# shaunplee/ray-tracing

Measured on AMD Instinct MI355X. Metric: Msamples/s (WxHxspp/s) + achieved HBM GB/s, final scene 1200x800x500spp, higher is better.
Workload: dtype f64

## Files before the change

include/rt_wide.h:

```cpp
#pragma once
#include <stdint.h>

#define RT_WIDE 4

typedef struct rt_wnode {
  float lo[3][RT_WIDE];
  float hi[3][RT_WIDE];
  int32_t child[RT_WIDE];
  int32_t pad[RT_WIDE];
} rt_wnode;

typedef struct rt_qnode {
  float origin[3];
  float scale[3];
  uint32_t qlo[3];
  uint32_t qhi[3];
  int32_t child[RT_WIDE];
} rt_qnode;

#define RT_WKEY_BITS 14
#define RT_WKEY_MASK ((1u << RT_WKEY_BITS) - 1u)
#define RT_WKEY_MAX_IDS (1 << (RT_WKEY_BITS - 1))
#define RT_WKEY_REJECTED 0x7f800000u

#if defined(__HIPCC__) || defined(__CUDACC__)
#define RT_WKEY_FN __host__ __device__ static inline
#else
#define RT_WKEY_FN static inline
#endif

RT_WKEY_FN int rt_wkey_fits(long long n_wide_nodes, long long n_leaf_slots) {
  return n_wide_nodes <= RT_WKEY_MAX_IDS && n_leaf_slots <= RT_WKEY_MAX_IDS;
}
RT_WKEY_FN int32_t rt_wkey_pack(uint32_t key_bits, int32_t ref) {
  return (int32_t)((key_bits & ~RT_WKEY_MASK) | ((uint32_t)ref & RT_WKEY_MASK));
}
RT_WKEY_FN int32_t rt_wkey_ref(int32_t word) {
  const uint32_t low = (uint32_t)word & RT_WKEY_MASK;
  return (int32_t)(low ^ (1u << (RT_WKEY_BITS - 1))) - (1 << (RT_WKEY_BITS - 1));
}

#ifdef __cplusplus
static_assert(sizeof(rt_wnode) == 128, "rt_wnode is 128 bytes");
static_assert(sizeof(rt_qnode) == 64, "rt_qnode is 64 bytes");
#endif
```

ray-tracing_amd/csrc/rt_kernels.h:

```cpp
#pragma once
#include <hip/hip_runtime.h>

#include <algorithm>
#include <cstdlib>
#include <cmath>
#include <cstdio>
#include <cstring>
#include <string>
#include <vector>

#include "rt.h"
#include "rt_device.h"
#include "rt_error.h"
#include "rt_internal.h"
#include "rt_trace.h"

using namespace rtd;

namespace {

struct UDiv {
  uint32_t m;
  int s1, s2;
};
// ... 481 lines not shown
          wq[1] = end2;
        }
      }
      if (w < 0) break;
      const uint32_t pid = (uint32_t)((long long)row * L.W + px);
      g.init(A.seed, pid, (uint32_t)s);
      g.reserve(3);
      const double ru = g.draw(), rv = g.draw();
      const int y = L.H - 1 - row;
      const double u = ((double)px + ru) / (double)L.W;
      const double v = ((double)y + rv) / (double)L.H;
      const Ray cray = get_ray(L.cam, u, v, g);
      t.ray.o = cray.o;
      t.ray.d = cray.d;
      t.ray.tm = cray.tm;
      thr = v3(1.0, 1.0, 1.0);
      depth = L.max_depth;
      if (depth <= 0) {
        end_sample(vmul(v3(1.0, 1.0, 1.0), v3(0.0, 0.0, 0.0)));
        continue;
      }
      start = true;
      if constexpr ((F & F_COUNT) != 0) ++segs;
    }
    if (start) {
      trav_begin<F>(t, plain(t.ray), S.world, kEps, INFINITY);
      if (S.ref_walk) trav_restart_ref(t, S.world, INFINITY);
      trav_media_first<F>(S, t, kEps, cnt, g, side);
      walking = true;
    }
    if (!walking) break;
    unsigned long long s1 = 0;
    if constexpr ((F & F_COUNT) != 0) s1 = stamp();
    const int live = __popcll(__ballot(true));
    const int stop = (live * A.trav_stop) >> 6;
    const int ls = (F & F_WIDE) ? A.leaf_stop : A.box_first;
    walk_until<F, PK>(S, t, walking, kEps, stk, stride, joint, stop, (live * ls) >> 6, cnt, g, side, A.med_batch);
    ready = !walking;
    if constexpr ((F & F_COUNT) != 0) {
      const unsigned long long s2 = stamp();
      ph_shade += s0b - s0;
      ph_setup += s1 - s0b;
      ph_trav += s2 - s1;
    }
  }
  if constexpr ((F & F_COUNT) != 0) {
    wave_add(&L.work[0], segs);
    wave_add(&L.work[1], cnt.box);
    wave_add(&L.work[2], cnt.prim);
    wave_add(&L.work[3], cnt.other);
    wave_add(&L.work[4], cnt.light);
    wave_add(&L.work[5], blocks);
    wave_add(&L.work[6], samples);
    wave_add(&L.work[7], cnt.wide);
    wave_add(&L.work[11], cnt.islot);
    wave_add(&L.work[12], cnt.lslot);
    wave_add(&L.work[13], cnt.oslot);
    wave_add(&L.work[14], cnt.phit);
    wave_add(&L.work[15], cnt.ties);
    if ((threadIdx.x & 63) == 0) {
      atomicAdd(&L.work[8], ph_setup);
      atomicAdd(&L.work[9], ph_trav);
      atomicAdd(&L.work[10], ph_shade);
    }
  }
}

template <unsigned F>
constexpr int lane_ints() {
  return ((F & (F_WIDE | F_MIXW)) ? RT_WSTACK : RT_STACK) + ((F & F_FRAMES) ? kSideInts : 0);
}

template <unsigned F, int WAVES>
__global__ void __launch_bounds__(RT_BLOCK, WAVES) render_philox2(RenderArgs A, int stack_entries) {
  extern __shared__ __attribute__((aligned(16))) int stk_mem[];
  __shared__ uint32_t wave_q[RT_BLOCK / 64][2];
  const LaunchConst& L = stage_const(A, stk_mem);
  __syncthreads();
  int* lane0 = &stk_mem[kLcBytes / 4 + threadIdx.x];
  philox_loop2<F>(A, L, A.S, lane0, RT_BLOCK, lane0 + stack_entries * RT_BLOCK,
                  wave_q[__builtin_amdgcn_readfirstlane(threadIdx.x >> 6)]);
}

template <unsigned F, int WAVES, bool LEAF_LDS = false, bool PK = false>
__global__ void __launch_bounds__(WAVES * 256, WAVES)
    render_philox2_lds(RenderArgs A, int n_nodes, int stack_entries, int n_leaves) {
  extern __shared__ __attribute__((aligned(16))) unsigned char lds0[];
  __shared__ uint32_t wave_q[WAVES * 4][2];
  constexpr int rec = (F & F_WIDE) ? (int)sizeof(rt_wnode) : (int)sizeof(rt_node);
  constexpr int lrec = (int)sizeof(rt_node);
  const LaunchConst& L = stage_const(A, lds0);
  unsigned char* lds = lds0 + kLcBytes;
  {
    const uint4* src = (F & F_WIDE) ? reinterpret_cast<const uint4*>(A.S.wnodes)
                                    : reinterpret_cast<const uint4*>(A.S.nodes);
    uint4* dst = reinterpret_cast<uint4*>(lds);
    const int n16 = n_nodes * (rec / 16);
    for (int i = threadIdx.x; i < n16; i += blockDim.x) dst[i] = src[i];
    const uint4* lsrc = reinterpret_cast<const uint4*>(A.S.leaves);
    uint4* ldst = reinterpret_cast<uint4*>(lds + (size_t)n_nodes * rec);
    const int l16 = n_leaves * (lrec / 16);
    for (int i = threadIdx.x; i < l16; i += blockDim.x) ldst[i] = lsrc[i];
  }
  __syncthreads();
  Scene S = A.S;
  if constexpr ((F & F_WIDE) != 0) S.wnodes = reinterpret_cast<const rt_wnode*>(lds);
  else S.nodes = reinterpret_cast<const rt_node*>(lds);
  if constexpr (LEAF_LDS) S.leaves = reinterpret_cast<const rt_node*>(lds + (size_t)n_nodes * rec);
  else n_leaves = 0;
  constexpr int lanes = WAVES * 256;
  unsigned char* lane_base = lds + (size_t)n_nodes * rec + (size_t)n_leaves * lrec;
  int* stk = reinterpret_cast<int*>(lane_base) + threadIdx.x;
  int* side_p = reinterpret_cast<int*>(lane_base + (size_t)stack_entries * lanes * sizeof(int)) + threadIdx.x;
  philox_loop2<F, PK>(A, L, S, stk, lanes, side_p, wave_q[__builtin_amdgcn_readfirstlane(threadIdx.x >> 6)]);
}

template <bool SKIP>
__device__ __forceinline__ void tail_body(const LaunchConst& A) {
  const long long j = (long long)blockIdx.x * 256 + threadIdx.x;
  if (j >= A.items_total - A.tail_start) return;
  int px, row, s0, s1;
  long long slot;
  if (!work_item<SKIP>(A, (uint32_t)(A.tail_start + j), px, row, s0, s1, slot)) return;
  const double* q = A.tail_buf + j * A.chunk * 3;
  V3 sum = v3(0, 0, 0);
  for (int k = 0; k < s1 - s0; ++k) sum = sum + v3(q[3 * k], q[3 * k + 1], q[3 * k + 2]);
  store_partial(A, slot, sum);
}
__global__ void __launch_bounds__(256) tail_combine(LaunchConst A) { tail_body<false>(A); }
__global__ void __launch_bounds__(256) tail_combine_skip(LaunchConst A) { tail_body<true>(A); }

template <bool MOMENTS, bool SKIP = false>
__device__ __forceinline__ void combine_body(const LaunchConst& A, double* moments) {
  const long long idx = (long long)blockIdx.x * 256 + threadIdx.x;
  if (idx >= A.slab) return;
  int px, row;
  if (!work_pixel(A, (uint32_t)idx, px, row)) return;
  if constexpr (SKIP) {
    if (skip_bit(A.skip, (uint32_t)idx)) return;
  }
  V3 acc = (A.combine & 1) ? vload(A.acc + idx * 3) : v3(0, 0, 0);
  V3 mom = v3(0, 0, 0);
  if constexpr (MOMENTS) {
    if (A.combine & 1) mom = vload(moments + idx * 3);
  }
  for (int k = 0; k < A.chunks; ++k) {
    const double* q = A.partial + ((long long)k * A.slab + idx) * 3;
    acc = acc + v3(q[0], q[1], q[2]);
    if constexpr (MOMENTS) {
      const int s0 = (A.chunk_base + k) * A.chunk;
      const double n = (double)(A.spp - s0 < A.chunk ? A.spp - s0 : A.chunk);
      mom = mom + v3((q[0] * q[0]) / n, (q[1] * q[1]) / n, (q[2] * q[2]) / n);
    }
  }
  if constexpr (MOMENTS) {
    moments[idx * 3 + 0] = mom.x;
    moments[idx * 3 + 1] = mom.y;
    moments[idx * 3 + 2] = mom.z;
  }
  if (A.combine & 2) {
    store_pixel(A, idx, divide(acc, (double)A.spp));
  } else {
    A.acc[idx * 3 + 0] = acc.x;
    A.acc[idx * 3 + 1] = acc.y;
    A.acc[idx * 3 + 2] = acc.z;
  }
// ... 579 lines not shown
  }
  if (w == 2) return (const void*)render_philox2_lds<V, 2, false, true>;
  if (w == 4) return (const void*)render_philox2_lds<V, 4, false, true>;
  if (w == 1) return (const void*)render_philox2_lds<V, 1, false, true>;
  return (const void*)render_philox2_lds<V, 3, false, true>;
}
template <unsigned V>
const void* pick_w(bool lds, int w, bool leaf_lds = false, bool q = false, bool pk = false) {
  if constexpr ((V & ~F_SKIP) == (kVarSpheres | F_WIDE)) {
    if (!lds && q) {
      if (w == 2) return (const void*)render_philox2<V | F_QNODE, 2>;
      if (w == 3) return (const void*)render_philox2<V | F_QNODE, 3>;
      if (w == 4) return (const void*)render_philox2<V | F_QNODE, 4>;
      return (const void*)render_philox2<V | F_QNODE, 1>;
    }
  }
  if constexpr ((V & F_WIDE) != 0 && (V & ~F_SKIP) != (kVarSpheres | F_WIDE)) {
    if (lds && pk) return pick_packed<V>(w, leaf_lds);
  }
  if constexpr ((V & F_WIDE) != 0) {
    if (lds && leaf_lds) {
      if (w == 4) return (const void*)render_philox2_lds<V, 4, true>;
      if (w == 2) return (const void*)render_philox2_lds<V, 2, true>;
      if (w == 3) return (const void*)render_philox2_lds<V, 3, true>;
    }
  }
  if (lds) {
    if (w == 2) return (const void*)render_philox2_lds<V, 2>;
    if (w == 4) return (const void*)render_philox2_lds<V, 4>;
    if (w == 1) return (const void*)render_philox2_lds<V, 1>;
    return (const void*)render_philox2_lds<V, 3>;
  }
  if (w == 2) return (const void*)render_philox2<V, 2>;
  if (w == 3) return (const void*)render_philox2<V, 3>;
  if (w == 4) return (const void*)render_philox2<V, 4>;
  return (const void*)render_philox2<V, 1>;
}
template <unsigned V>
const void* pick(int loop, bool lds, int w, bool count, bool leaf_lds, bool q = false, bool skip = false,
                 bool pk = false) {
  if constexpr ((V & F_SKIP) == 0) {
    if (skip) return count ? nullptr : pick<V | F_SKIP>(loop, lds, w, false, leaf_lds, q, false, pk);
    if (count) {
      if constexpr (V == kVarSpheres) {
        if (loop == 2 && q) return (const void*)render_philox2<V | F_WIDE | F_COUNT | F_QNODE, 1>;
      }
      if (loop == 2) return (const void*)render_philox2<V | F_WIDE | F_COUNT, 1>;
      return loop ? (const void*)render_philox2<V | F_COUNT, 1> : (const void*)render_philox<V | F_COUNT, 1>;
    }
  }
  if (loop == 2) return pick_w<V | F_WIDE>(lds, w, leaf_lds, q, pk);
  if (loop == 1) return pick_w<V>(lds, w);
  if (lds) {
    if (w == 2) return (const void*)render_philox_lds<V, 2>;
    if (w == 4) return (const void*)render_philox_lds<V, 4>;
    if (w == 1) return (const void*)render_philox_lds<V, 1>;
    return (const void*)render_philox_lds<V, 3>;
  }
  if (w == 2) return (const void*)render_philox<V, 2>;
  if (w == 3) return (const void*)render_philox<V, 3>;
  if (w == 4) return (const void*)render_philox<V, 4>;
  return (const void*)render_philox<V, 1>;
}
template <unsigned V>
const void* pick_full(int loop, bool lds, int w, bool count, bool skip = false) {
  if constexpr ((V & F_SKIP) == 0) {
    if (skip) return count ? nullptr : pick_full<V | F_SKIP>(loop, lds, w, false);
    if (count) return loop ? (const void*)render_philox2<V | F_COUNT, 1> : (const void*)render_philox<V | F_COUNT, 1>;
  }
  if (loop) {
    if (lds) return w >= 3 ? (const void*)render_philox2_lds<V, 3> : (const void*)render_philox2_lds<V, 2>;
    if (w >= 4) return (const void*)render_philox2<V, 4>;
    return w >= 3 ? (const void*)render_philox2<V, 3> : (const void*)render_philox2<V, 2>;
  }
  return w >= 2 ? (const void*)render_philox<V, 2> : (const void*)render_philox<V, 1>;
}

}

namespace rt {
const void* philox_kernel_spheres(int loop, bool lds, int w, bool count, bool leaf_lds, bool q, bool skip, bool pk);
const void* philox_kernel_spheres_global(int w, bool skip);
const void* philox_kernel_spheres_packed(int w, bool leaf_lds, bool skip);
const void* philox_kernel_cornell(int loop, bool lds, int w, bool count, bool leaf_lds, bool skip, bool pk);
const void* philox_kernel_full(int loop, bool lds, int w, bool count, bool skip);
const void* philox_kernel_full_dark(int loop, bool lds, int w, bool count, bool skip);
}
```

ray-tracing_amd/csrc/rt_render.hip:

```cpp
#include <rccl/rccl.h>

#include <numeric>
#include <vector>

#include "rt_frame_blob.h"
#include "rt_kernels.h"
#include "rt_prepare.h"


struct rt_ctx {
  int device = 0;
  int cu_count = 0;
  int blocks_per_cu = 0;
  hipStream_t stream = nullptr;
  hipEvent_t ev0 = nullptr, ev1 = nullptr;
  hipEvent_t ev_done = nullptr;
  hipStream_t last_stream = nullptr;
  rt_node* d_nodes = nullptr;
  DMat* d_mats = nullptr;
  rt_texture* d_texs = nullptr;
  rt_perlin* d_perlins = nullptr;
  rt_image* d_images = nullptr;
  uint8_t* d_pool = nullptr;
  Scene scene{};
// ... 383 lines not shown
    R.S = A.S;
    R.lc = d_lc;
    R.seed = A.seed;
    R.flags = A.flags;
    R.trav_stop = A.trav_stop;
    R.leaf_stop = A.leaf_stop;
    R.box_first = A.box_first;
    R.med_batch = A.med_batch;
    R.prof = A.prof;
    if (units_of(slab * per_batch) >= (1ll << 32) - (1ll << 24))
      return invalid("image too large: more than 2^32 - 2^24 work units per shard and launch");
    const size_t need_tail = (size_t)std::min(slab * per_batch, tail_items) * (size_t)A.chunk * 3 * sizeof(double);
    if (need_tail > c->tail_bytes) {
      HIPCHK(hipEventSynchronize(c->ev_done));
      (void)hipFree(c->d_tail);
      c->d_tail = nullptr;
      c->tail_bytes = 0;
      ++c->allocs;
      HIPCHK(hipMalloc((void**)&c->d_tail, need_tail));
      c->tail_bytes = need_tail;
    }
    A.tail_buf = c->d_tail;
    for (int b0 = 0; b0 < chunks_total; b0 += per_batch) {
      const int nk = std::min(per_batch, chunks_total - b0);
      const int k0 = span_first + b0;
      fill_batch_geometry(A, k0, nk, tail_items);
      const bool last = b0 + nk == chunks_total;
      A.combine = (k0 > 0 ? 1 : 0) | (last && !span.keep ? 2 : 0);
      {
        LaunchConst B = A;
        void* sargs[] = {&B, &d_lc};
        HIPCHK(hipLaunchKernel((const void*)launch_setup, dim3(1), dim3(64), sargs, 0, st));
        HIPCHK(hipGetLastError());
      }
      if (b0 == 0) HIPCHK(hipEventRecord(ev_begin, st));
      HIPCHK(hipLaunchKernel(fn, grid, block, args, bytes, st));
      HIPCHK(hipGetLastError());
      if (A.tail_start < A.items_total) {
        LaunchConst B = A;
        void* targs[] = {&B};
        HIPCHK(hipLaunchKernel(A.skip ? (const void*)tail_combine_skip : (const void*)tail_combine, dim3((unsigned)((A.items_total - A.tail_start + 255) / 256)),
                               dim3(256), targs, 0, st));
        HIPCHK(hipGetLastError());
      }
      if (last) HIPCHK(hipEventRecord(ev_end, st));
      const int rc = launch_combine(c, A, st, span.moments);
      if (rc) return rc;
    }
    return RT_OK;
  };
  const char* stop_env = std::getenv("RTAMD_TRAV_STOP");
  {
    const char* be = std::getenv("RTAMD_BATCH");
    A.batch = be ? std::max(1, std::min(4096, std::atoi(be))) : 1024;
    const double waves = (double)c->cu_count * 4 * 4;
    A.batch_per_item = (float)(1.0 / (16.0 * waves));
    const char* bf = std::getenv("RTAMD_BATCH_FLOOR");
    A.batch_floor = bf ? std::max(0, std::min(1024, std::atoi(bf))) : (is_full(variant_for(c->features)) ? 0 : 64);
  }
  A.trav_stop = stop_env ? std::max(0, std::min(63, std::atoi(stop_env)))
                         : (c->n_nodes > 20000 ? 16 : 8);
  const char* leaf_env = std::getenv("RTAMD_LEAF_STOP");
  A.leaf_stop = leaf_env ? std::max(0, std::min(64, std::atoi(leaf_env))) : A.trav_stop;
  const char* box_env = std::getenv("RTAMD_BOX_FIRST");
  A.box_first = box_env ? std::max(0, std::min(64, std::atoi(box_env))) : 4;
  const char* med_env = std::getenv("RTAMD_MED_BATCH");
  A.med_batch = med_env ? std::max(0, std::min(64, std::atoi(med_env))) : 0;
  A.rev_tiles = env_off("RTAMD_TILE_REV") || !std::getenv("RTAMD_TILE_REV") ? 0u : (uint32_t)per_shard;
  const unsigned var = variant_for(c->features);
  const bool count = d_work != nullptr;
  const bool skip = A.skip != nullptr;
  if (skip && count) return invalid("the counting build has no adaptive-frame kernels");
  const bool replace = c->replace_ok && !env_off("RTAMD_REPLACE");
  const char* wenv = std::getenv("RTAMD_WIDE");
  const bool want_wide = wenv ? wenv[0] != '0' : c->rebuilt_bvh;
  const bool wide = replace && c->d_wnodes && !(A.flags & RT_FLAG_REFERENCE_CULL) && want_wide && !is_full(var);
  const int loop = wide ? 2 : (replace ? 1 : 0);
  if (loop && is_full(var)) {
    const char* te = std::getenv("RTAMD_TAIL");
    tail_items = (long long)c->cu_count * (te ? std::max(0, std::min(1 << 16, std::atoi(te))) : 768);
  }
  int waves = (var == kVarSpheres || loop) ? waves_target(3) : waves_target(is_full(var) ? 2 : 1);
  const int side_ints = side_ints_of(var, c->scene.frames, loop) + (lane_lds_of(var, loop) ? 4 : 0);
  if (!count && !env_off("RTAMD_LDS") && (!is_full(var) || loop)) {
    const int entries = wide ? c->wide_stack_need + 3 : c->stack_need + 2;
    const int items = wide ? c->n_wnodes : c->n_nodes;
    const size_t rec = wide ? sizeof(rt_wnode) : sizeof(rt_node);
    const bool leaf_lds = wide && !env_off("RTAMD_LEAF_LDS");
    auto lds_bytes = [&](int w, int& n_leaves) {
      const size_t b =
          (size_t)kLcBytes + (size_t)items * rec + (size_t)(entries + side_ints) * (w * 256) * sizeof(int);
      n_leaves = leaf_lds && b + (size_t)c->n_leaves * sizeof(rt_node) <= kLdsBudget ? c->n_leaves : 0;
      return b + (size_t)n_leaves * sizeof(rt_node);
    };
    int n_leaves = 0;
    if (var == kVarSpheres && !std::getenv("RTAMD_WAVES") && lds_bytes(4, n_leaves) <= kLdsBudget &&
        (!leaf_lds || n_leaves > 0) && A.work_total >= (long long)c->cu_count * 1024)
      waves = 4;
    const int block = waves * 256;
    const size_t bytes = lds_bytes(waves, n_leaves);
    if (bytes <= kLdsBudget) {
      const bool pk = wide && wide_keys_packed(c);
      const void* fn = philox_kernel(var, loop, true, waves, false, skip, n_leaves > 0, false, pk);
      c->last_wide_packed = pk;
      HIPCHK(hipFuncSetAttribute(fn, hipFuncAttributeMaxDynamicSharedMemorySize, (int)bytes));
      int n_items = items;
      void* args[] = {&R, &n_items, (void*)&entries, &n_leaves};
      c->last_launch = rt_launch_info{var | (loop == 2 ? F_WIDE : 0u) | (skip ? F_SKIP : 0u), loop, 1, n_leaves > 0, waves, c->cu_count,
                                      block, (int)bytes, A.work_total, A.chunk,
                                      (loop == 2 || (loop == 1 && c->mixed_wide)) ? c->n_wnodes : 0, batches, 0};
      return run(fn, dim3(c->cu_count), dim3(block), bytes, args);
    }
  }
  const void* fn = philox_kernel(var, loop, false, count ? 1 : waves, count, skip, false, loop == 2 && c->d_qnodes);
  c->last_wide_packed = 0;
  int entries = wide ? c->wide_stack_need + 3 : c->stack_need + 2;
  const size_t dyn = loop ? (size_t)kLcBytes + (size_t)(entries + side_ints) * RT_BLOCK * sizeof(int) : 0;
  if (loop) HIPCHK(hipFuncSetAttribute(fn, hipFuncAttributeMaxDynamicSharedMemorySize, (int)dyn));
  int bpc = 1;
  HIPCHK(hipOccupancyMaxActiveBlocksPerMultiprocessor(&bpc, fn, RT_BLOCK, dyn));
  const long long want = (A.work_total + RT_BLOCK - 1) / RT_BLOCK;
  const long long resident = (long long)c->cu_count * std::max(1, bpc);
  const int grid = (int)std::max(1ll, std::min(want, resident));
  c->last_launch = rt_launch_info{var | (loop == 2 ? F_WIDE : 0u) | (count ? F_COUNT : 0u) | (skip ? F_SKIP : 0u), loop, 0, 0,
                                  count ? 1 : waves, grid, RT_BLOCK, (int)dyn, A.work_total, A.chunk,
                                  (loop == 2 || (loop == 1 && c->mixed_wide)) ? c->n_wnodes : 0, batches, 0};
  void* args[] = {&R, &entries};
  return run(fn, dim3(grid), dim3(RT_BLOCK), dyn, args);
}

int render_multi(rt_ctx* c, const rt_camera* cam, rt_render_params p, uint8_t* out_rgb, double* out_lin) {
  const int n = 1 + (int)c->peers.size();
  p.shard_count = n;
  int tile, tiles_x;
  long long tt, ps, slab;
  geometry(&p, tile, tiles_x, tt, ps, slab);
  auto dev_ctx = [&](int r) { return r == 0 ? c : c->peers[r - 1]; };
  const long long npx = (long long)p.width * p.height;
  int rc = RT_OK;
  for (int r = 0; r < n && !rc; ++r) {
    rt_ctx* d = dev_ctx(r);
    DEVICE_SCOPE(d->device);
    if ((rc = grow(d, d->fb_slab, (size_t)slab * 3))) break;
    if (out_lin && (rc = grow(d, d->fb_slab_lin, sizeof(double) * (size_t)slab * 3))) break;
  }
  {
    DEVICE_SCOPE(c->device);
    if (!rc) rc = grow(c, c->fb_gather, (size_t)n * slab * 3);
    if (!rc && out_lin) rc = grow(c, c->fb_gather_lin, sizeof(double) * (size_t)n * slab * 3);
    if (!rc) rc = grow(c, c->fb_img, (size_t)npx * 3);
    if (!rc && out_lin) rc = grow(c, c->fb_img_lin, sizeof(double) * (size_t)npx * 3);
  }
  if (rc) return rc;
  void* gathered = c->fb_gather.p;
  void* gathered_lin = c->fb_gather_lin.p;
  void* img = c->fb_img.p;
  void* img_lin = c->fb_img_lin.p;
  for (int r = 0; r < n; ++r) {
    rt_ctx* d = dev_ctx(r);
    DEVICE_SCOPE(d->device);
    rt_render_params pr = p;
    pr.shard_rank = r;
    if ((rc = launch_philox(d, cam, &pr, r, n, (uint8_t*)d->fb_slab.p, out_lin ? (double*)d->fb_slab_lin.p : nullptr,
                            d->stream)))
      return rc;
    if (r == 0) HIPCHK(hipEventRecord(c->ev_gather, c->stream));
  }
  {
    DeviceGuard _dg(c->device);
    NCCLCHK(ncclGroupStart());
    for (int r = 0; r < n; ++r) {
      rt_ctx* d = dev_ctx(r);
      const ncclResult_t g = ncclGather(d->fb_slab.p, r == 0 ? gathered : nullptr, (size_t)slab * 3, ncclUint8, 0,
                                        c->comms[r], d->stream);
      const ncclResult_t gl = g == ncclSuccess && out_lin
                                  ? ncclGather(d->fb_slab_lin.p, r == 0 ? gathered_lin : nullptr, (size_t)slab * 3,
                                               ncclFloat64, 0, c->comms[r], d->stream)
                                  : g;
      if (gl != ncclSuccess) {
        (void)ncclGroupEnd();
        return nccl_fail(gl, "ncclGather");
      }
    }
    NCCLCHK(ncclGroupEnd());
  }
  {
    DEVICE_SCOPE(c->device);
    HIPCHK(hipEventRecord(c->ev_gathered, c->stream));
    if ((rc = rt_assemble_async(c, &p, (const uint8_t*)gathered, (uint8_t*)img, c->stream))) return rc;
    if (out_lin && (rc = rt_assemble_linear_async(c, &p, (const double*)gathered_lin, (double*)img_lin, c->stream)))
      return rc;
    HIPCHK(hipEventRecord(c->ev_asm, c->stream));
  }
  for (int r = 0; r < n; ++r) {
    rt_ctx* d = dev_ctx(r);
    DEVICE_SCOPE(d->device);
    HIPCHK(hipStreamSynchronize(d->stream));
  }
// ... 1288 lines not shown
```

ray-tracing_amd/csrc/rt_trace.h:

```cpp
#pragma once
#include "rt_device.h"

namespace rtd {

template <unsigned F>
constexpr bool kRay32 = (F & (F_WIDE | F_MIXW)) != 0;
template <unsigned F>
constexpr bool kNoInv = (F & F_WIDE) != 0 && (F & (F_ALL | F_MIXW)) == 0;

struct Cnt {
  unsigned box, prim, other, light, wide;
  unsigned islot, lslot, oslot;
  unsigned phit;
  unsigned ties;
  unsigned long long* prof;
};
enum : unsigned { K_BOX = 1u, K_WIDE = 2u, K_LEAF = 4u, K_MEDIUM = 8u, K_FRAME = 16u };

__device__ __forceinline__ int hmod256(long long a) {
  const long long r = a % 256;
  return (int)(r < 0 ? r + 256 : r);
}
__device__ inline double noise(const rt_perlin* P, double sc, V3 p) {
  const V3 q = scale(sc, p);
// ... 829 lines not shown

__device__ __forceinline__ void wide_keys2(const Trav& t, f32x2 nx, f32x2 ny, f32x2 nz, f32x2 fx, f32x2 fy, f32x2 fz,
                                           float& k0, float& k1) {
  const f32x2 ox = {t.o32x, t.o32x}, oy = {t.o32y, t.o32y}, oz = {t.o32z, t.o32z};
  const f32x2 ix = {t.i32x, t.i32x}, iy = {t.i32y, t.i32y}, iz = {t.i32z, t.i32z};
  const f32x2 tnx = (nx - ox) * ix, tny = (ny - oy) * iy, tnz = (nz - oz) * iz;
  const f32x2 tfx = (fx - ox) * ix, tfy = (fy - oy) * iy, tfz = (fz - oz) * iz;
  const float n0 = fmaxf(fmaxf(tnx.x, tny.x), fmaxf(tnz.x, t.tmin32));
  const float n1 = fmaxf(fmaxf(tnx.y, tny.y), fmaxf(tnz.y, t.tmin32));
  const float f0 = fminf(fminf(tfx.x, tfy.x), fminf(tfz.x, t.tmax32));
  const float f1 = fminf(fminf(tfx.y, tfy.y), fminf(tfz.y, t.tmax32));
  const bool h0 = n0 * (1.0f - 0x1p-21f) <= fmaf(f0, 1.0f + 0x1p-21f, t.slack);
  const bool h1 = n1 * (1.0f - 0x1p-21f) <= fmaf(f1, 1.0f + 0x1p-21f, t.slack);
  k0 = h0 ? fminf(n0, 3.0e38f) : INFINITY;
  k1 = h1 ? fminf(n1, 3.0e38f) : INFINITY;
}

__device__ __forceinline__ void cswap(float& ka, int& ca, float& kb, int& cb) {
  const bool s = kb < ka;
  const float k = s ? kb : ka;
  const int c = s ? cb : ca;
  kb = s ? ka : kb;
  cb = s ? ca : cb;
  ka = k;
  ca = c;
}

__device__ __forceinline__ void pswap(int& a, int& b) {
  const int lo = min(a, b);
  b = max(a, b);
  a = lo;
}

__device__ __forceinline__ float4 qplanes(uint32_t q, float s, float o) {
  return float4{fmaf((float)(q & 255u), s, o), fmaf((float)((q >> 8) & 255u), s, o),
                fmaf((float)((q >> 16) & 255u), s, o), fmaf((float)(q >> 24), s, o)};
}

template <unsigned F = 0, bool PK = false>
__device__ __forceinline__ bool wide_node(const Scene& S, Trav& t, int* stk, int stride, int w) {
  float4 nx, ny, nz, fx, fy, fz;
  int4 ch;
  if constexpr ((F & F_QNODE) != 0) {
    const uint4* qb = reinterpret_cast<const uint4*>(&S.qnodes[w]);
    const uint4 a = qb[0], b = qb[1], c = qb[2];
    const uint4 d = qb[3];
    ch = int4{(int)d.x, (int)d.y, (int)d.z, (int)d.w};
    const float ox = __uint_as_float(a.x), oy = __uint_as_float(a.y), oz = __uint_as_float(a.z);
    const float sx = __uint_as_float(a.w), sy = __uint_as_float(b.x), sz = __uint_as_float(b.y);
    const bool mx = signbit(t.i32x), my = signbit(t.i32y), mz = signbit(t.i32z);
    nx = qplanes(mx ? c.y : b.z, sx, ox);
    fx = qplanes(mx ? b.z : c.y, sx, ox);
    ny = qplanes(my ? c.z : b.w, sy, oy);
    fy = qplanes(my ? b.w : c.z, sy, oy);
    nz = qplanes(mz ? c.w : c.x, sz, oz);
    fz = qplanes(mz ? c.x : c.w, sz, oz);
  } else {
    const float* base = reinterpret_cast<const float*>(&S.wnodes[w]);
    const int ox = signbit(t.i32x) ? 12 : 0, oy = signbit(t.i32y) ? 16 : 4, oz = signbit(t.i32z) ? 20 : 8;
    nx = *reinterpret_cast<const float4*>(base + ox);
    ny = *reinterpret_cast<const float4*>(base + oy);
    nz = *reinterpret_cast<const float4*>(base + oz);
    fx = *reinterpret_cast<const float4*>(base + (ox ^ 12));
    fy = *reinterpret_cast<const float4*>(base + (oy < 12 ? oy + 12 : oy - 12));
    fz = *reinterpret_cast<const float4*>(base + (oz < 12 ? oz + 12 : oz - 12));
    ch = *reinterpret_cast<const int4*>(base + 24);
  }
  float k0, k1, k2, k3;
  wide_keys2(t, f32x2{nx.x, nx.y}, f32x2{ny.x, ny.y}, f32x2{nz.x, nz.y}, f32x2{fx.x, fx.y}, f32x2{fy.x, fy.y},
             f32x2{fz.x, fz.y}, k0, k1);
  wide_keys2(t, f32x2{nx.z, nx.w}, f32x2{ny.z, ny.w}, f32x2{nz.z, nz.w}, f32x2{fx.z, fx.w}, f32x2{fy.z, fy.w},
             f32x2{fz.z, fz.w}, k2, k3);
  int c0 = ch.x, c1 = ch.y, c2 = ch.z, c3 = ch.w;
  const int n_hit = (k0 < INFINITY) + (k1 < INFINITY) + (k2 < INFINITY) + (k3 < INFINITY);
  if constexpr (PK) {
    int p0 = rt_wkey_pack(__float_as_uint(k0), c0), p1 = rt_wkey_pack(__float_as_uint(k1), c1);
    int p2 = rt_wkey_pack(__float_as_uint(k2), c2), p3 = rt_wkey_pack(__float_as_uint(k3), c3);
    pswap(p0, p1);
    pswap(p2, p3);
    pswap(p0, p2);
    pswap(p1, p3);
    pswap(p1, p2);
    c0 = rt_wkey_ref(p0);
    c1 = rt_wkey_ref(p1);
    c2 = rt_wkey_ref(p2);
    c3 = rt_wkey_ref(p3);
  } else {
    cswap(k0, c0, k1, c1);
    cswap(k2, c2, k3, c3);
    cswap(k0, c0, k2, c2);
    cswap(k1, c1, k3, c3);
    cswap(k1, c1, k2, c2);
  }
  const int e0 = n_hit > 3 ? c3 : (n_hit > 2 ? c2 : c1);
  const int e1 = n_hit > 3 ? c2 : c1;
  stk[t.sp * stride] = e0;
  stk[(t.sp + 1) * stride] = e1;
  stk[(t.sp + 2) * stride] = c1;
  t.sp += n_hit > 1 ? n_hit - 1 : 0;
  t.node = c0;
  return n_hit != 0;
}

constexpr int kNone = (int)0x80000000;

template <unsigned F>
__device__ __forceinline__ bool trav_pop_mixed(const Scene& S, Trav& t, const int* stk, int stride, Side& side,
                                               double t_min = kEps) {
  bool reb = false;
  for (;;) {
    const bool end = t.sp == 0;
    const int e = end ? 0 : stk[(--t.sp) * stride];
    const bool frame = (F & F_FRAMES) && ((F & F_MIXW) ? (e >= 0 && (e & RT_FRAME)) : (e & RT_FRAME));
    if (end || !frame) {
      if ((F & F_FRAMES) && reb) {
        Ray pr = side.get_ray();
        for (int k = 0; k < t.level; ++k) pr = enter_instance(&S.nodes[side.frame(k)], pr);
        t.ray = prep(pr);
        if constexpr ((F & F_MIXW) != 0) set_ray32(t, t_min);
      }
      t.node = e;
      return !end;
    }
    --t.level;
    reb = true;
  }
}

template <unsigned F, class R>
__device__ __forceinline__ bool trav_step(const Scene& S, Trav& t, double t_min, int* stk, int stride, bool joint,
                                          Cnt& cnt, R& g, Side& side) {
  bool wide = false;
  if constexpr ((F & F_WIDE) != 0) wide = !t.ref;
  if (wide) {
    if (t.node >= 0) {
      if constexpr ((F & F_COUNT) != 0) ++cnt.wide;
      if (wide_node<F>(S, t, stk, stride, t.node)) return true;
    } else {
      const rt_node* n = &S.leaves[~t.node];
      trav_leaf<F>(S, t, n, ~t.node | kSlotTag, t_min, cnt, g, side, false);
    }
    if (t.sp == 0) return false;
    t.node = stk[(--t.sp) * stride];
    return true;
  }
  bool leaf_slot = false, to_wide = false;
  if constexpr ((F & F_MIXW) != 0) {
    to_wide = t.node >= 0 && (t.node & RT_WNODE);
    leaf_slot = t.node < 0;
  }
  if (!to_wide) {
  int id = leaf_slot ? (~(t.node | RT_ISMED) | kSlotTag) : (t.node & ~(RT_SUB | RT_IDTAGS));
  int tag = leaf_slot ? RT_SUB : (kRefMixed<F> ? (t.node & RT_SUB) : 0);
  bool refsem = t.ref && !tag;
  const rt_node* n = leaf_slot ? &S.leaves[~(t.node | RT_ISMED)] : &S.nodes[id];
  const int tf = n->type;
  const int type = tf & RT_TYPE_MASK;
  if (type == RT_NODE_BVH) {
   constexpr int kFuse = (F & F_WIDE) ? 0 : 8;
   for (int fuse = 0;; ++fuse) {
    if (fuse) {
      id = t.node & ~(RT_SUB | RT_IDTAGS);
      tag = kRefMixed<F> ? (t.node & RT_SUB) : 0;
      refsem = t.ref && !tag;
      n = &S.nodes[id];
    }
    const bool same = kRefMixed<F> && (t.node & RT_IDTAGS) == RT_SAMEBOX;
    if constexpr ((F & F_COUNT) != 0) cnt.box += !same;
    if (same || box_hit(n->f, t.ray, t_min, refsem ? t.closest : closest_up<F>(t), joint)) {
      const int c = n->c;
      const bool ord = (c & RT_BVH_ORDERED) && !t.redo;
      if constexpr ((F & F_MIXW) != 0) {
        if (ord && (c & RT_WROOT)) {
          t.node = RT_WNODE | ((c >> 2) & RT_WROOT_MASK);
          to_wide = true;
          break;
        }
      }
      const bool flip = ord && !(c & RT_BVH_MEDIA_FIRST) && comp(t.ray.d, c & 3) < 0;
      const int ctag = (kRefMixed<F> && ord) ? RT_SUB : tag;
      stk[(t.sp++) * stride] = (flip ? n->a : n->b) | ctag;
      t.node = (flip ? n->b : n->a) | ctag;
      if ((t.node & RT_ISBOX) && fuse < kFuse) continue;
      return true;
    }
    break;
   }
  } else if ((F & F_FRAMES) && (type == RT_NODE_TRANSLATE || type == RT_NODE_ROTATE) && !(tf & RT_CHAIN_PRIM)) {
    if (t.level == 0) side.put_ray(plain(t.ray));
    Ray cr = plain(t.ray);
    int cur = leaf_slot ? n->c : id, ct = tf;
    if ((F & F_MIXW) && leaf_slot && (tf & RT_FRAME_FUSED)) {
      rt_node rec;
      {
        const uint4* q = reinterpret_cast<const uint4*>(n);
        const uint4 q0 = q[0], q1 = q[1], q2 = q[2], q3 = q[3];
        uint4* r = reinterpret_cast<uint4*>(&rec);
        r[0] = q0, r[1] = q1, r[2] = q2, r[3] = q3;
      }
      cur = rec.c;
      if constexpr ((F & F_COUNT) != 0) ++cnt.other;
      side.frame(t.level++) = cur;
      stk[(t.sp++) * stride] = RT_FRAME | cur;
      cr = enter_instance(&rec, cr);
      if (tf & RT_FRAME_FUSED2) {
        if constexpr ((F & F_COUNT) != 0) ++cnt.other;
        side.frame(t.level++) = rec.a;
        stk[(t.sp++) * stride] = RT_FRAME | rec.a;
        const int ax = (tf >> RT_FRAME_AX2_SHIFT) & 3;
        cr = Ray{unrotate_point(ax, rec.f[3], rec.f[4], cr.o), unrotate_point(ax, rec.f[3], rec.f[4], cr.d), cr.tm};
      }
      const int inner = (int)rec.f[5];
      t.ray = prep(cr);
      set_ray32(t, t_min);
      t.node = (inner & RT_WNODE) ? inner : (inner | tag);
      return true;
    } else {
      do {
        if constexpr ((F & F_COUNT) != 0) ++cnt.other;
        side.frame(t.level++) = cur;
        stk[(t.sp++) * stride] = RT_FRAME | cur;
        cr = enter_instance(&S.nodes[cur], cr);
        cur = S.nodes[cur].a;
        ct = S.nodes[cur].type;
      } while (((ct & RT_TYPE_MASK) == RT_NODE_TRANSLATE || (ct & RT_TYPE_MASK) == RT_NODE_ROTATE) &&
               !(ct & RT_CHAIN_PRIM));
    }
    t.ray = prep(cr);
    if constexpr ((F & F_MIXW) != 0) set_ray32(t, t_min);
    t.node = cur | tag;
    return true;
  } else {
    trav_leaf<F>(S, t, n, id, t_min, cnt, g, side, refsem);
  }
  if (!to_wide) return trav_pop_mixed<F>(S, t, stk, stride, side, t_min);
  }
  if constexpr ((F & F_MIXW) != 0) {
    if constexpr ((F & F_COUNT) != 0) ++cnt.wide;
    refresh_ray32(t);
    if (wide_node<F>(S, t, stk, stride, t.node & ~RT_WNODE)) return true;
  }
  return trav_pop_mixed<F>(S, t, stk, stride, side, kEps);
}


__device__ __forceinline__ int trav_pop(Trav& t, const int* stk, int stride) {
  return t.sp ? stk[(--t.sp) * stride] : kNone;
}
__device__ __forceinline__ void trav_postpone(Trav& t, int* stk, int stride) {
  if (t.node < 0 && t.node != kNone && t.pend < 0) {
    t.pend = ~t.node;
    t.node = trav_pop(t, stk, stride);
  }
}
template <unsigned F, bool PK = false>
__device__ __forceinline__ void wide_inner(const Scene& S, Trav& t, int* stk, int stride, Cnt& cnt) {
  if constexpr ((F & F_COUNT) != 0) ++cnt.wide;
  if (!wide_node<F, PK>(S, t, stk, stride, t.node)) t.node = trav_pop(t, stk, stride);
  trav_postpone(t, stk, stride);
}
template <unsigned F, class R>
__device__ __forceinline__ void wide_leaf(const Scene& S, Trav& t, double t_min, int* stk, int stride, Cnt& cnt, R& g,
                                          Side& side) {
  for (int k = 0; k < 1 && t.pend >= 0; ++k) {
    const rt_node* n = &S.leaves[t.pend];
    trav_leaf<F>(S, t, n, t.pend | kSlotTag, t_min, cnt, g, side, false);
    t.pend = -1;
  }
  trav_postpone(t, stk, stride);
}

template <unsigned F, bool PK = false, class R>
__device__ __forceinline__ void walk_until(const Scene& S, Trav& t, bool& walking, double t_min, int* stk, int stride,
                                           bool joint, int stop, int leaf_stop, Cnt& cnt, R& g, Side& side,
                                           int med_batch = 0) {
  if constexpr ((F & F_WIDE) == 0) {
    for (;;) {
      const int n_walk = __popcll(__ballot(walking));
      if (n_walk <= stop) break;
      constexpr bool kBoxFirst = kRefMixed<F>;
      const bool box_id = walking && t.node >= 0 && (t.node & (RT_ISBOX | RT_WNODE));
      const bool at_box = kBoxFirst && box_id;
      int ty = -1;
      if constexpr ((F & F_COUNT) != 0) {
        if (walking) {
          if ((F & F_MIXW) && t.node < 0) ty = S.leaves[~(t.node | RT_ISMED)].type & RT_TYPE_MASK;
          else if (box_id) ty = RT_NODE_BVH;
          else ty = S.nodes[t.node & ~(RT_SUB | RT_IDTAGS)].type & RT_TYPE_MASK;
        }
      }
      bool go = walking;
      if constexpr (kBoxFirst) {
        const int n_box = __popcll(__ballot(at_box));
        if (leaf_stop < n_walk && n_box > leaf_stop) {
          go = walking && at_box;
        } else if ((F & F_MEDIA) && med_batch > 0) {
          const bool at_med = walking && t.node >= 0 && (t.node & (RT_WNODE | RT_IDTAGS)) == RT_ISMED;
          const int n_med = __popcll(__ballot(at_med));
          if (n_med < med_batch && n_med < n_walk) go = walking && !at_med;
        }
      }
      if constexpr ((F & F_COUNT) != 0) {
        ++cnt.islot;
        const bool inst = ty == RT_NODE_TRANSLATE || ty == RT_NODE_ROTATE;
        const bool box = ty == RT_NODE_BVH;
        cnt.lslot += (__ballot(go && box) != 0) + (__ballot(go && inst) != 0) +
                     (__ballot(go && ty == RT_NODE_CONSTANT_MEDIUM) != 0) +
                     (__ballot(go && !box && !inst && ty != RT_NODE_CONSTANT_MEDIUM) != 0);
      }
      unsigned kinds = 0;
      unsigned long long t0 = 0;
      if constexpr ((F & F_COUNT) != 0) {
        const bool wide = walking && t.node >= 0 && (t.node & RT_WNODE);
        const bool inst = ty == RT_NODE_TRANSLATE || ty == RT_NODE_ROTATE;
        bool frame = false;
        if (inst) {
          const int nid = t.node < 0 ? -1 : (t.node & ~(RT_SUB | RT_IDTAGS));
          const int tf = t.node < 0 ? S.leaves[~(t.node | RT_ISMED)].type : S.nodes[nid].type;
          frame = !(tf & RT_CHAIN_PRIM);
        }
        kinds = (__ballot(go && ty == RT_NODE_BVH && !wide) ? K_BOX : 0u) | (__ballot(go && wide) ? K_WIDE : 0u) |
                (__ballot(go && ty == RT_NODE_CONSTANT_MEDIUM) ? K_MEDIUM : 0u) | (__ballot(go && frame) ? K_FRAME : 0u) |
                (__ballot(go && ty >= 0 && ty != RT_NODE_BVH && ty != RT_NODE_CONSTANT_MEDIUM && !frame) ? K_LEAF : 0u);
        t0 = stamp();
      }
      if (go) walking = trav_step<F>(S, t, t_min, stk, stride, joint, cnt, g, side);
      if constexpr ((F & F_COUNT) != 0) {
        const unsigned long long t1 = stamp();
        if (cnt.prof && __lane_id() == (unsigned)(__ffsll((long long)__ballot(true)) - 1)) {
          atomicAdd(&cnt.prof[kinds], t1 - t0);
          atomicAdd(&cnt.prof[32 + kinds], 1ull);
        }
      }
    }
  } else {
    for (;;) {
      if (__popcll(__ballot(walking)) <= stop) break;
      const bool seeking = walking && (t.ref || (t.pend < 0 && t.node >= 0));
      const bool holding = walking && !t.ref && t.pend >= 0;
      unsigned kinds = 0;
      unsigned long long t0 = 0;
      if constexpr ((F & F_COUNT) != 0) t0 = stamp();
      if (__popcll(__ballot(seeking)) > leaf_stop || __ballot(holding) == 0) {
        if constexpr ((F & F_COUNT) != 0) {
          ++cnt.islot;
          kinds = __ballot(walking && t.ref) ? K_BOX | K_WIDE : K_WIDE;
        }
        if (walking && t.ref) {
          walking = trav_step<F>(S, t, t_min, stk, stride, joint, cnt, g, side);
        } else if (walking && t.node >= 0) {
          wide_inner<F, PK>(S, t, stk, stride, cnt);
          walking = t.node != kNone || t.pend >= 0;
        }
      } else {
        if constexpr ((F & F_COUNT) != 0) {
          ++cnt.lslot;
          kinds = K_LEAF;
        }
        if (holding) {
          wide_leaf<F>(S, t, t_min, stk, stride, cnt, g, side);
          walking = t.node != kNone || t.pend >= 0;
        }
      }
      if constexpr ((F & F_COUNT) != 0) {
        const unsigned long long t1 = stamp();
        if (cnt.prof && __lane_id() == (unsigned)(__ffsll((long long)__ballot(true)) - 1)) {
          atomicAdd(&cnt.prof[kinds], t1 - t0);
          atomicAdd(&cnt.prof[32 + kinds], 1ull);
        }
      }
    }
  }
}

template <unsigned F>
__device__ __forceinline__ bool trav_finish(const Scene& S, const Trav& t, const Ray& r, double t_min, Hit& h,
                                            const Side& side) {
  if (t.best_node < 0) return false;
  const bool slot = (F & (F_WIDE | F_MIXW)) && (t.best_node & kSlotTag);
  const rt_node* n = slot ? &S.leaves[t.best_node & ~kSlotTag] : &S.nodes[t.best_node];
  int levels = 0;
  if constexpr ((F & F_FRAMES) != 0) levels = t.best_level;
  Ray fr = r;
  int sub = t.best_sub;
  const rt_node* leaf = n;
  int chain_id = -1, chain_len = 0;
  if constexpr ((F & F_FRAMES) != 0)
    for (int k = 0; k < levels; ++k) fr = enter_instance(&S.nodes[side.best(k)], fr);
  bool med = false;
  if constexpr ((F & F_MEDIA) != 0) med = sub == kSubMedium;
  if (med) {
    h.t = t.closest;
    h.p = at(fr, t.closest);
    h.n = v3(1, 0, 0);
    h.u = 0;
    h.v = 0;
    h.ff = 1;
    h.mat = n->b;
  }
  if constexpr ((F & F_INST) != 0) {
    if (!med && (sub & kSubChain)) {
      sub &= ~kSubChain;
      chain_id = slot ? n->c : t.best_node;
      int cur = chain_id;
      while ((S.nodes[cur].type & RT_TYPE_MASK) == RT_NODE_TRANSLATE || (S.nodes[cur].type & RT_TYPE_MASK) == RT_NODE_ROTATE) {
        fr = enter_instance(&S.nodes[cur], fr);
        cur = S.nodes[cur].a;
        ++chain_len;
      }
      leaf = &S.nodes[cur];
    }
  }
  if (!med) prim_record<F>(S, leaf, sub, fr, t.closest, h);
  for (int lv = levels + chain_len - 1; lv >= 0; --lv) {
    Ray rl = r;
    const rt_node* inst = nullptr;
    int cur = chain_id;
    for (int k = 0; k <= lv; ++k) {
      if ((F & F_FRAMES) && k < levels) {
        inst = &S.nodes[side.best(k)];
      } else {
        inst = &S.nodes[cur];
        cur = inst->a;
      }
      rl = enter_instance(inst, rl);
    }
    exit_instance(inst, rl, h);
  }
  return true;
}

template <unsigned F, int D>
__device__ __forceinline__ double htbl_pdf_value(const Scene& S, int id, V3 origin, V3 v, const RayX& r) {
  id &= ~RT_IDTAGS;
  const rt_node* n = &S.nodes[id];
  const int type = n->type & RT_TYPE_MASK;
  Hit hh;
  if (type == RT_NODE_RECT_XZ) {
    if (!rect_hit(1, n->f[0], n->f[1], n->f[2], n->f[3], n->f[4], n->a, r, kEps, INFINITY, hh)) return 0.0;
    const double area = (n->f[1] - n->f[0]) * (n->f[3] - n->f[2]);
    const double distance_squared = hh.t * hh.t * sqlen(v);
    const double cosine = fabs(dot(v, hh.n) / vlen(v));
    return distance_squared / (cosine * area);
// ... 152 lines not shown
```

Measured before the change: 5243.

## Keep packed distance keys on the wide stack and cull stale entries after leaf hits

The wide traversal now pushes packed key+ref words onto the stack and decodes the ref only on pop. After a leaf hit shrinks tmax, it pops every top-of-stack entry whose stored entry distance lies beyond the new bound, so those subtrees are never revisited. A counting-build kernel variant for the packed path is also added and selected when the count mode fits the LDS budget. This adds a float compare loop per leaf hit and relies on conservative slack to avoid culling nodes that could still hold a hit.

```diff
diff --git a/include/rt_wide.h b/include/rt_wide.h
--- a/include/rt_wide.h
+++ b/include/rt_wide.h
@@ -40,6 +40,13 @@
   return (int32_t)(low ^ (1u << (RT_WKEY_BITS - 1))) - (1 << (RT_WKEY_BITS - 1));
 }
 
+RT_WKEY_FN int rt_wkey_beyond(int32_t word, float tmax32, float slack) {
+  const uint32_t kb = (uint32_t)word & ~RT_WKEY_MASK;
+  float key;
+  __builtin_memcpy(&key, &kb, sizeof key);
+  return key * (1.0f - 0x1p-21f) > __builtin_fmaf(tmax32, 1.0f + 0x1p-21f, slack);
+}
+
 #ifdef __cplusplus
 static_assert(sizeof(rt_wnode) == 128, "rt_wnode is 128 bytes");
 static_assert(sizeof(rt_qnode) == 64, "rt_qnode is 64 bytes");
diff --git a/ray-tracing_amd/csrc/rt_k_count_packed.hip b/ray-tracing_amd/csrc/rt_k_count_packed.hip
--- /dev/null
+++ b/ray-tracing_amd/csrc/rt_k_count_packed.hip
@@ -0,0 +1,9 @@
+#define RT_PHILOX_OPAQUE_KEY 1
+#include "rt_kernels.h"
+
+namespace rt {
+const void* philox_kernel_count_packed(unsigned var) {
+  if (var == kVarSpheres) return (const void*)render_philox2_count_packed<kVarSpheres | F_WIDE | F_COUNT>;
+  return (const void*)render_philox2_count_packed<kVarCornell | F_WIDE | F_COUNT>;
+}
+}
diff --git a/ray-tracing_amd/csrc/rt_kernels.h b/ray-tracing_amd/csrc/rt_kernels.h
--- a/ray-tracing_amd/csrc/rt_kernels.h
+++ b/ray-tracing_amd/csrc/rt_kernels.h
@@ -587,6 +587,18 @@
                   wave_q[__builtin_amdgcn_readfirstlane(threadIdx.x >> 6)]);
 }
 
+template <unsigned F>
+__global__ void __launch_bounds__(RT_BLOCK, 1) render_philox2_count_packed(RenderArgs A, int stack_entries) {
+  static_assert((F & F_WIDE) != 0 && (F & F_COUNT) != 0, "the 4-wide counting build only");
+  extern __shared__ __attribute__((aligned(16))) int stk_mem[];
+  __shared__ uint32_t wave_q[RT_BLOCK / 64][2];
+  const LaunchConst& L = stage_const(A, stk_mem);
+  __syncthreads();
+  int* lane0 = &stk_mem[kLcBytes / 4 + threadIdx.x];
+  philox_loop2<F, true>(A, L, A.S, lane0, RT_BLOCK, lane0 + stack_entries * RT_BLOCK,
+                        wave_q[__builtin_amdgcn_readfirstlane(threadIdx.x >> 6)]);
+}
+
 template <unsigned F, int WAVES, bool LEAF_LDS = false, bool PK = false>
 __global__ void __launch_bounds__(WAVES * 256, WAVES)
     render_philox2_lds(RenderArgs A, int n_nodes, int stack_entries, int n_leaves) {
@@ -1332,6 +1344,7 @@
 const void* philox_kernel_spheres(int loop, bool lds, int w, bool count, bool leaf_lds, bool q, bool skip, bool pk);
 const void* philox_kernel_spheres_global(int w, bool skip);
 const void* philox_kernel_spheres_packed(int w, bool leaf_lds, bool skip);
+const void* philox_kernel_count_packed(unsigned var);
 const void* philox_kernel_cornell(int loop, bool lds, int w, bool count, bool leaf_lds, bool skip, bool pk);
 const void* philox_kernel_full(int loop, bool lds, int w, bool count, bool skip);
 const void* philox_kernel_full_dark(int loop, bool lds, int w, bool count, bool skip);
diff --git a/ray-tracing_amd/csrc/rt_render.hip b/ray-tracing_amd/csrc/rt_render.hip
--- a/ray-tracing_amd/csrc/rt_render.hip
+++ b/ray-tracing_amd/csrc/rt_render.hip
@@ -489,7 +489,8 @@
   }
   int waves = (var == kVarSpheres || loop) ? waves_target(3) : waves_target(is_full(var) ? 2 : 1);
   const int side_ints = side_ints_of(var, c->scene.frames, loop) + (lane_lds_of(var, loop) ? 4 : 0);
-  if (!count && !env_off("RTAMD_LDS") && (!is_full(var) || loop)) {
+  bool count_pk = false;
+  if (!env_off("RTAMD_LDS") && (!is_full(var) || loop)) {
     const int entries = wide ? c->wide_stack_need + 3 : c->stack_need + 2;
     const int items = wide ? c->n_wnodes : c->n_nodes;
     const size_t rec = wide ? sizeof(rt_wnode) : sizeof(rt_node);
@@ -506,7 +507,9 @@
       waves = 4;
     const int block = waves * 256;
     const size_t bytes = lds_bytes(waves, n_leaves);
-    if (bytes <= kLdsBudget) {
+    if (count) {
+      count_pk = bytes <= kLdsBudget && wide && wide_keys_packed(c);
+    } else if (bytes <= kLdsBudget) {
       const bool pk = wide && wide_keys_packed(c);
       const void* fn = philox_kernel(var, loop, true, waves, false, skip, n_leaves > 0, false, pk);
       c->last_wide_packed = pk;
@@ -519,8 +522,9 @@
       return run(fn, dim3(c->cu_count), dim3(block), bytes, args);
     }
   }
-  const void* fn = philox_kernel(var, loop, false, count ? 1 : waves, count, skip, false, loop == 2 && c->d_qnodes);
-  c->last_wide_packed = 0;
+  const void* fn = count_pk ? rt::philox_kernel_count_packed(var)
+                            : philox_kernel(var, loop, false, count ? 1 : waves, count, skip, false, loop == 2 && c->d_qnodes);
+  c->last_wide_packed = count_pk;
   int entries = wide ? c->wide_stack_need + 3 : c->stack_need + 2;
   const size_t dyn = loop ? (size_t)kLcBytes + (size_t)(entries + side_ints) * RT_BLOCK * sizeof(int) : 0;
   if (loop) HIPCHK(hipFuncSetAttribute(fn, hipFuncAttributeMaxDynamicSharedMemorySize, (int)dyn));
diff --git a/ray-tracing_amd/csrc/rt_trace.h b/ray-tracing_amd/csrc/rt_trace.h
--- a/ray-tracing_amd/csrc/rt_trace.h
+++ b/ray-tracing_amd/csrc/rt_trace.h
@@ -935,9 +935,9 @@
     pswap(p1, p3);
     pswap(p1, p2);
     c0 = rt_wkey_ref(p0);
-    c1 = rt_wkey_ref(p1);
-    c2 = rt_wkey_ref(p2);
-    c3 = rt_wkey_ref(p3);
+    c1 = p1;
+    c2 = p2;
+    c3 = p3;
   } else {
     cswap(k0, c0, k1, c1);
     cswap(k2, c2, k3, c3);
@@ -1097,30 +1097,41 @@
 }
 
 
+template <bool PK = false>
 __device__ __forceinline__ int trav_pop(Trav& t, const int* stk, int stride) {
-  return t.sp ? stk[(--t.sp) * stride] : kNone;
-}
+  if constexpr (PK) {
+    return t.sp ? rt_wkey_ref(stk[(--t.sp) * stride]) : kNone;
+  } else {
+    return t.sp ? stk[(--t.sp) * stride] : kNone;
+  }
+}
+template <bool PK = false>
 __device__ __forceinline__ void trav_postpone(Trav& t, int* stk, int stride) {
   if (t.node < 0 && t.node != kNone && t.pend < 0) {
     t.pend = ~t.node;
-    t.node = trav_pop(t, stk, stride);
+    t.node = trav_pop<PK>(t, stk, stride);
   }
 }
 template <unsigned F, bool PK = false>
 __device__ __forceinline__ void wide_inner(const Scene& S, Trav& t, int* stk, int stride, Cnt& cnt) {
   if constexpr ((F & F_COUNT) != 0) ++cnt.wide;
-  if (!wide_node<F, PK>(S, t, stk, stride, t.node)) t.node = trav_pop(t, stk, stride);
-  trav_postpone(t, stk, stride);
-}
-template <unsigned F, class R>
+  if (!wide_node<F, PK>(S, t, stk, stride, t.node)) t.node = trav_pop<PK>(t, stk, stride);
+  trav_postpone<PK>(t, stk, stride);
+}
+template <unsigned F, bool PK = false, class R>
 __device__ __forceinline__ void wide_leaf(const Scene& S, Trav& t, double t_min, int* stk, int stride, Cnt& cnt, R& g,
                                           Side& side) {
   for (int k = 0; k < 1 && t.pend >= 0; ++k) {
     const rt_node* n = &S.leaves[t.pend];
+    [[maybe_unused]] const float bound_before = t.tmax32;
     trav_leaf<F>(S, t, n, t.pend | kSlotTag, t_min, cnt, g, side, false);
     t.pend = -1;
-  }
-  trav_postpone(t, stk, stride);
+    if constexpr (PK && (F & F_RECT) == 0) {
+      if (t.tmax32 < bound_before)
+        while (t.sp && rt_wkey_beyond(stk[(t.sp - 1) * stride], t.tmax32, t.slack)) --t.sp;
+    }
+  }
+  trav_postpone<PK>(t, stk, stride);
 }
 
 template <unsigned F, bool PK = false, class R>
@@ -1211,7 +1222,7 @@
           kinds = K_LEAF;
         }
         if (holding) {
-          wide_leaf<F>(S, t, t_min, stk, stride, cnt, g, side);
+          wide_leaf<F, PK>(S, t, t_min, stk, stride, cnt, g, side);
           walking = t.node != kNone || t.pend >= 0;
         }
       }
```

After: 5304, median of 6. 1.2% higher.
